# liuyuan-pal/Gen6D

Measured on AMD Instinct MI355X. Metric: query images/sec (detect+select+3x refine), 64 ref views, higher is better.
Workload: dtype f32

## Files before the change

### gen6d_amd/lib.py

```python
import ctypes as C
import os

_HERE = os.path.dirname(os.path.abspath(__file__))
LIB_PATH = os.path.join(_HERE, "libgen6d_hip.so")

G6D_ERRORS = {-1: "G6D_EINVAL", -2: "G6D_ENOSPC", -3: "G6D_ELAUNCH"}


class G6dWinoSeg(C.Structure):
    _fields_ = [("in_", C.c_void_p), ("out_full", C.c_void_p), ("out_pool", C.c_void_p),
                ("N", C.c_int32), ("H", C.c_int32), ("W", C.c_int32), ("ld_in", C.c_int32), ("ld_full", C.c_int32), ("ld_pool", C.c_int32)]


class G6dConv16Seg(C.Structure):
    _fields_ = [("in_", C.c_void_p), ("out_full", C.c_void_p), ("out_pool", C.c_void_p),
                ("N", C.c_int32), ("D", C.c_int32), ("H", C.c_int32), ("W", C.c_int32), ("ld_in", C.c_int32), ("ld_full", C.c_int32),
                ("ld_pool", C.c_int32)]


class G6dRange16(C.Structure):
    _fields_ = [("exps", C.c_void_p), ("rec", C.c_void_p), ("slot_in", C.c_int32), ("slot_out", C.c_int32)]


class G6dCorrSeg(C.Structure):
# ... 77 lines not shown
    "g6d_conv16_direct_plan": [_P, _I, _I, _P, _I, _I, _I, _I, _I, _I, _P, _I],
    "g6d_affine_split16_to": [_P, _I, _P, _P, _I, _I, _I, _I, _I, _I, _I, _P, _I, _I, _I, _I, _P, _P],
    "g6d_upsample_bilinear_split16": [_P, _I, _P, _P, _I, _I, _I, _I, _I, _I, _P, _I, _I, _I, _I, _P, _P],
    "g6d_l2norm_split16": [_P, _I, _I, _I, _P, _I, _P, _P],
    "g6d_vgg_conv1_pool_nhwc_norm": [_P, _I, _I, _I, _P, _P, _I, _I, _P, _P, _P, _P],
    "g6d_wino_conv3x3": [_P, _I, _I, _I, _I, _I, _P, _P, _I, _I, _P, _I, _P, _I, _P, C.c_size_t, _P],
    "g6d_wino_conv3x3_multi": [_P, _I, _I, _P, _P, _I, _I, _P, C.c_size_t, _P],
    "g6d_wino16_conv3x3_multi": [_P, _I, _I, _P, _P, _I, _I, _I, _P, C.c_size_t, _P],
    "g6d_wino43_conv3x3_multi": [_P, _I, _I, _P, _P, _I, _I, _P, C.c_size_t, _P],
    "g6d_corr2d_wino43_multi": [_P, _I, _I, _P, _I, _I, _P, C.c_size_t, _P],
    "g6d_l2norm_rows": [_P, _I, _I, _I, _P],
    "g6d_nchw_to_nhwc": [_P, _I, _I, _I, _I, _I, _P, _I, _P],
    "g6d_selector_ref_sums": [_P, _I, _I, _I, _P, _P, _P],
    "g6d_selector_prod_affine": [_P, _P, _P, _I, _I, _I, _D, _P, _P, _P],
    "g6d_selector_scan": [_P, _P, _I, _I, _I, _P, _P, _P],
    "g6d_selector_levels": [_I, _I, _P, _P, _P, _P, _P, _I, _I, _I, _D, _P, _P, _P, _P, _P],
    "g6d_refiner_volume": [_P, _P, _P, _P, _I, _I, _I, _I, _I, _I, _I, _P, _P, _P],
    "g6d_refiner_volume_kp": [_P, _P, _P, _P, _P, _P, _I, _I, _I, _I, _I, _I, _I, _P, _P, _I, _P],
    "g6d_refiner_volume_kp_pairs": [_P, _P, _P, _P, _P, _P, _I, _I, _I, _I, _I, _I, _I, _P, _P, _I, _P, _P, _P],
    "g6d_detector_assemble": [_P, _P, _P, _I, _I, _I, C.POINTER(C.c_float), _F, _I, _I, _I, _I, _P, _I, _P],
    "g6d_detector_score_mlp_max": [_P, _I, _I, _I, _P, _P, _P, _P, _P, _P],
    "g6d_detector_decode": [_P, _I, _P, _I, _P, _I, _I, _I, _I, _P, _I, _P],
    "g6d_resize_bilinear_pyramid": [_P, _I, _I, _I, _I, C.POINTER(C.c_int), C.POINTER(C.c_int), C.POINTER(C.c_void_p), _P],
    "g6d_zero_bytes": [_P, C.c_size_t, _P],
    "g6d_vps_norm": [_P, _I, _P, _I, _I, _I, _P],
    "g6d_max_an_add": [_P, _I, _I, _I, _I, _P, _P, _I, _I, _P],
    "g6d_attention": [_P, _P, _P, _I, _I, _I, _I, _P, _I, _I, _P],
    "g6d_layernorm": [_P, _I, _I, _I, _P, _P, _F, _P, _I, _P],
    "g6d_affine_act_add": [_P, _I, _P, _P, _I, _P, _I, _I, _I, _P, _I, _I, _P],
    "g6d_linear_gemv": [_P, _I, _I, _P, _P, _I, _I, _P, _P],
    "g6d_linear_gemv_batch": [_P, _I, _I, _P, _P, _I, _I, _P, _P, C.c_size_t, _P],
    "g6d_chain_crop_from_detection": [_P, _F, _P, _I, _P],
    "g6d_chain_pose_from_selection": [_P, _P, _P, _I, _P, _P, _P, _P, _P, _P, _I, _P],
    "g6d_chain_refine_prepare": [_P, _P, _P, _F, _F, _P, _P, _I, _I, _P, _P, _F, _P, _I, _P],
    "g6d_chain_refine_update": [_P, _P, _P, _P, _I, _P, _P, _I, _P],
    "g6d_warp_batch": [_P, _P, _P, _I, _I, _I, _I, _P, _P, _I, _I, _P],
    "g6d_warp_perspective": [_P, _I, _I, _I, C.POINTER(C.c_float), _P, _I, _I, _I, _F, _P],
    "g6d_track_gather": [_P, _P, _P, _P, _I, _P],
    "g6d_track_commit": [_P, _P, _P, _I, _P, _I, _F, _P, _P, _P, _P, _P, _I, _P],
    "g6d_track_gate": [_P, _P, _P, _P, _I, _P],
    "g6d_track_health": [_P, _P, _P, _P, _I, _I, _P, _I, _P, _D, _I, _D, _D, _D, _D, _D, _D, _P, _P, _P, _P, _I, _P],
    "g6d_track_verify": [_P, _P, _P, _P, _P, _D, _D, _D, _D, _I, _P, _P, _I, _P],
    "g6d_frame_ingest": [_P, _I, _P, _I, _I, _I, _P, _P],
    "g6d_sizeof_frame_desc": [],
    "g6d_frame_ingest_mesh": [_P, _P, _I, _P, _I, _I, _I, _P, _P],
    "g6d_sizeof_mesh_desc": [],
    "g6d_track_corners": [_P, _P, _P, _P, _P, _P, _I, _P],
    "g6d_frame_emit": [_P, _I, _P, _I, _I, _I, _P, _P, _P],
    "g6d_sizeof_sink_desc": [],
    "g6d_frame_emit_source": [_P, _I, _P, _I, _P, _P, _I, _I, _I, _I, _P],
    "g6d_frame_crop": [_P, _P, _P, _I, _I, _I, _P, _P, _I, _I, _P],
    "g6d_frame_ingest_area": [_P, _P, _I, _P, _I, _I, _I, _P, _P],
    "g6d_frame_crop_area": [_P, _P, _P, _I, _I, _I, _P, _P, _I, _I, _I, _P],
}

_lib = None


def load():
    global _lib
    if _lib is not None:
        return _lib
    if not os.path.exists(LIB_PATH):
        raise RuntimeError(f"{LIB_PATH} is missing: build it with `python __graft_entry__.py` "
                           "(make -C gen6d_amd/csrc). There is no fallback path.")
    import torch
    lib = C.CDLL(LIB_PATH)
    for name, args in SIGNATURES.items():
        fn = getattr(lib, name)
        fn.argtypes = args
        fn.restype = C.c_int
    lib.g6d_abi_version.restype = C.c_int
    lib.g6d_sizeof_conv_desc.restype = C.c_int
    if lib.g6d_sizeof_conv_desc() != C.sizeof(G6dConv):
        raise RuntimeError("libgen6d_hip.so: G6dConv layout differs from the ctypes binding (stale build?)")
    if lib.g6d_sizeof_frame_desc() != C.sizeof(G6dFrame):
        raise RuntimeError("libgen6d_hip.so: G6dFrame layout differs from the ctypes binding (stale build?)")
    if lib.g6d_sizeof_mesh_desc() != C.sizeof(G6dMesh):
        raise RuntimeError("libgen6d_hip.so: G6dMesh layout differs from the ctypes binding (stale build?)")
    if lib.g6d_sizeof_sink_desc() != C.sizeof(G6dSink):
        raise RuntimeError("libgen6d_hip.so: G6dSink layout differs from the ctypes binding (stale build?)")
    lib.g6d_last_error.restype = C.c_char_p
    lib.g6d_set_knob.argtypes, lib.g6d_set_knob.restype = [C.c_char_p, C.c_double], C.c_int
    lib.g6d_get_knob.argtypes, lib.g6d_get_knob.restype = [C.c_char_p], C.c_double
    lib.g6d_reset_knobs.argtypes, lib.g6d_reset_knobs.restype = [], None
    _lib = lib
    return lib


def set_knob(name, value):
    check(load().g6d_set_knob(name.encode(), float(value)), f"g6d_set_knob({name})")


def get_knob(name):
    return load().g6d_get_knob(name.encode())


def reset_knobs():
    load().g6d_reset_knobs()


def check(rc, what):
    if rc != 0:
        msg = load().g6d_last_error().decode()
        raise RuntimeError(f"{what} failed: {G6D_ERRORS.get(rc, rc)} ({msg})")
```

### gen6d_amd/network/detector.py

```python
import numpy as np
import torch
import torch.nn.functional as F

from .. import ops, parallel, specs
from .backbone import (is_16bit, pack_trunk, trunk_features, trunk_features_multi, trunk_route, winograd43_corr_filters,
                       winograd43_corr_filters_padded)
from .params import ParamBank, fold_vgg

_TAPS = ("c5", "c7_pre", "p7")
MAX_BATCH = 16


class Detector(ParamBank):
    default_cfg = {
        "vgg_score_stats": [[36.264317, 13.151907], [13910.291, 5345.965], [829.70807, 387.98788]],
        "vgg_score_max": 10,
        "detection_scales": [-1.0, -0.5, 0.0, 0.5],
        "train_feats": False,
    }

    def __init__(self, cfg):
        self.cfg = {**self.default_cfg, **cfg}
        super().__init__(specs.detector_rows())
        if len(self.cfg["detection_scales"]) != 4:
            raise NotImplementedError("score_conv expects 3 levels x 4 detection scales (12 channels)")
        self.pool_ratio = 8
        self.ref_center_feats = None
        self.ref_wino15_43 = None
        self.ref_wino7_43 = None
        self._corr16 = {}
        self.ref_shape = None
        self.rank, self.world, self.group = 0, 1, None
        self.sharded = False

    def set_shard(self, rank, world, group=None, force_collectives=False):
        self.rank, self.world, self.group = int(rank), int(world), group
        self.sharded = self.world > 1 or bool(force_collectives)

    def _pack(self):
        if self._packed is None:
            pk = {"vgg": pack_trunk(fold_vgg(self, "backbone.features"))}
            w0, b0 = self.conv_w("score_conv.0")
            w1, b1 = self.conv_w("score_conv.2")
            pk["mlp"] = (w0.reshape(64, 12).contiguous(), b0, w1.reshape(64, 64).contiguous(), b1)
            heads = ("score_predict", "scale_predict", "offset_predict")
            l0 = [self.conv_w(f"{h}.0") for h in heads]
            pk["h0"] = (torch.cat([w for w, _ in l0], 0).contiguous(), torch.cat([b for _, b in l0], 0).contiguous())
            pk["h1"] = [self.conv_w(f"{h}.2") for h in heads]
            l2 = [self.conv_w(f"{h}.4") for h in heads]
            w4 = torch.zeros((sum(w.shape[0] for w, _ in l2), 9, 192), dtype=torch.float32, device=l2[0][0].device)
            row = 0
            for i, (w, _) in enumerate(l2):
                w4[row:row + w.shape[0], :, 64 * i:64 * i + 64] = w
                row += w.shape[0]
            pk["h2"] = (w4.contiguous(), torch.cat([b for _, b in l2], 0).contiguous())
            self._packed = pk
        return self._packed

    def extract_feats(self, imgs):
        return trunk_features(self._pack()["vgg"], imgs, _TAPS, False)

    def load_impl(self, ref_imgs):
        b, e = parallel.shard_range(ref_imgs.shape[0], self.rank, self.world)
        if e == b:
            raise ValueError("more ranks than reference views")
        ref_imgs = F.interpolate(ref_imgs[b:e], size=(120, 120))
        feats = self.extract_feats(ref_imgs)
        self.ref_center_feats = [f.reshape(f.shape[0], f.shape[2] * f.shape[3], 512).contiguous() for f in feats]
        self.ref_ksize = [f.shape[2] for f in feats]
        self._corr16 = {}
        self.ref_shape = [120, 120]
        wino43 = self.ref_center_feats[0].shape[0] % 32 == 0
        self.ref_wino15_43 = winograd43_corr_filters(self.ref_center_feats[0], 15) if wino43 else None
        self.ref_wino7_43 = winograd43_corr_filters_padded(self.ref_center_feats[1], 7)[0] if wino43 else None

    def _corr16_filters(self, level, mode):
        if (level, mode) not in self._corr16:
            self._corr16[level, mode] = ops.corr16_pack(self.ref_center_feats[level], mode)
        return self._corr16[level, mode]

    def corr_routes(self, hq, wq):
        sizes = [self._scale_size(hq, wq, sc) for sc in self.cfg["detection_scales"]]
        trunk16 = trunk_route(self._pack()["vgg"], sizes, _TAPS, f43=True, pairs=self.pairs_on) == "direct"
        rfn = self.ref_center_feats[0].shape[0]
        routes = []
        for k in self.ref_ksize:
            if k in (15, 7) and trunk16 and rfn == 32:
                routes.append("corr16")
            elif k in (15, 7) and rfn % 32 == 0 and not ops.MATH_MODE:
                routes.append("wino43")
            else:
                routes.append("patch" if rfn <= 32 else "conv")
        return routes

    def _scores_one_scale(self, que_img, scale_idx, stacked, hs, ws):
        self._scores_from_feats(self.extract_feats(que_img), scale_idx, stacked, hs, ws)

    def _scores_from_pyramid(self, feats, routes, scale_ids, stacked, hs, ws):
        rfn = self.ref_center_feats[0].shape[0]
        dev = stacked.device
        qn = feats[0][0].shape[0]
        maps = [[None] * 3 for _ in feats]
        for l, (wref, k, route) in enumerate(zip(self.ref_center_feats, self.ref_ksize, routes)):
            xs = [f[l] for f in feats]
            assert is_16bit(xs[0]) == (route == "corr16"), "the trunk did not hand the level over in the format of its route"
            if route == "corr16":
                mode = 3 if len(xs[0].shape) == 5 else (1 if xs[0].dtype == torch.bfloat16 else 2)
                filt = self._corr16_filters(l, mode)
                outs = [torch.empty((qn, 1, x.shape[1], x.shape[2], rfn), dtype=torch.float32, device=dev) for x in xs]
                ops.corr16_multi(xs, filt, outs)
                for i, o in enumerate(outs):
                    maps[i][l] = o.reshape(qn * o.shape[2] * o.shape[3], rfn)
                continue
            lo = min(x.data_ptr() for x in xs)
            hi = max(x.data_ptr() + x.numel() * 4 for x in xs)
            if hi - lo >= (1 << 31) or not all(x.is_contiguous() for x in xs):
                seg = ops.alloc_like_segments([tuple(x.shape) for x in xs], dev)
                for d_, x in zip(seg, xs):
                    d_.copy_(x)
                xs = seg
            if route == "conv":
                outs = [torch.empty((qn, 1, x.shape[2], x.shape[3], rfn), dtype=torch.float32, device=dev) for x in xs]
                for x, o in zip(xs, outs):
                    ops.conv(x, wref, None, o, ksize=(1, k, k), pad=(0, k // 2, k // 2))
            else:
                outs = ops.alloc_like_segments([(qn, 1, x.shape[2], x.shape[3], rfn) for x in xs], dev)
                if route == "patch":
                    ops.corr2d_patch_multi(xs, wref, outs, k)
                elif k == 15:
                    ops.corr2d_wino43_multi([x.contiguous() for x in xs], self.ref_wino15_43, outs, 5)
                else:
                    ops.corr2d_wino43_multi([x.contiguous() for x in xs], self.ref_wino7_43, outs, 3, k_true=7)
            for i, o in enumerate(outs):
                maps[i][l] = o.reshape(qn * o.shape[2] * o.shape[3], rfn)
        for f, si, m in zip(feats, scale_ids, maps):
            hc, wc = (f[0].shape[1], f[0].shape[2]) if is_16bit(f[0]) else (f[0].shape[2], f[0].shape[3])
            ops.detector_assemble(m[0], m[1], m[2], hc, wc, self.cfg["vgg_score_stats"],
                                  float(self.cfg["vgg_score_max"]), hs, ws, si, stacked, batch=qn)

    def _scores_from_feats(self, feats, scale_idx, stacked, hs, ws):
        x0, x1, x2 = feats
        rfn = self.ref_center_feats[0].shape[0]
        qn = x0.shape[0]
        maps = []
        for x, wref, k in zip((x0, x1, x2), self.ref_center_feats, self.ref_ksize):
            _, _, h, w, _ = x.shape
            o = torch.empty((qn, 1, h, w, rfn), dtype=torch.float32, device=x.device)
            if k >= 7 and rfn <= 32 and qn == 1:
                ops.corr2d_patch(x, wref, o, k)
            else:
                ops.conv(x, wref, None, o, ksize=(1, k, k), pad=(0, k // 2, k // 2))
            maps.append(o.reshape(qn * h * w, rfn))
        hc, wc = x0.shape[2], x0.shape[3]
        ops.detector_assemble(maps[0], maps[1], maps[2], hc, wc, self.cfg["vgg_score_stats"],
                              float(self.cfg["vgg_score_max"]), hs, ws, scale_idx, stacked, batch=qn)

    @staticmethod
    def _scale_size(hq, wq, scale):
        ht, wt = int(np.round(hq * 2 ** scale)), int(np.round(wq * 2 ** scale))
        if ht % 32 != 0: ht = (ht // 32 + 1) * 32
        if wt % 32 != 0: wt = (wt // 32 + 1) * 32
        return ht, wt

    def _detect_batch(self, que_imgs, multi=True):
        pk = self._pack()
        qn, _, hq, wq = que_imgs.shape
        hs, ws = hq // 8, wq // 8
        dev = que_imgs.device
        rfn = self.ref_center_feats[0].shape[0]
        P = hs * ws
        stacked = torch.empty((qn * P, rfn, 12), dtype=torch.float32, device=dev)
        def resized(scale):
            return F.interpolate(que_imgs, size=self._scale_size(hq, wq, scale), mode="bilinear")

        order = sorted(enumerate(self.cfg["detection_scales"]), key=lambda t: -t[1])
        if multi:
            pyr = ops.resize_bilinear_pyramid(que_imgs, [self._scale_size(hq, wq, sc) for _, sc in order])
            routes = self.corr_routes(hq, wq)
            t16 = tuple(tap for tap, r in zip(_TAPS, routes) if r == "corr16")
            feats = trunk_features_multi(pk["vgg"], pyr, _TAPS, f43=True, taps16=t16, rng=self._pair_rng(), pairs=self.pairs_on)
            self._scores_from_pyramid(feats, routes, [si for si, _ in order], stacked, hs, ws)
        else:
            ops.fork_join([(lambda si=si, sc=sc: self._scores_one_scale(resized(sc), si, stacked, hs, ws)) for si, sc in order], dev)
        feats = ops.detector_score_mlp_max(stacked, *pk["mlp"])
        if self.sharded:
            parallel.all_reduce_(feats, "max", self.group)
        k3, p3 = (1, 3, 3), (0, 1, 1)
        a = torch.empty((qn, 1, hs, ws, 192), dtype=torch.float32, device=dev)
        ops.conv(feats.view(qn, 1, hs, ws, 64), pk["h0"][0], pk["h0"][1], a, ksize=k3, pad=p3, out_act=1)
        b = torch.empty_like(a)
        o4 = torch.empty((qn, 1, hs, ws, 4), dtype=torch.float32, device=dev)
        for i in range(3):
            w1, b1 = pk["h1"][i]
            ops.conv(a[..., 64 * i:64 * i + 64], w1, b1, b[..., 64 * i:64 * i + 64], ksize=k3, pad=p3, out_act=1)
        ops.conv(b, pk["h2"][0], pk["h2"][1], o4, ksize=k3, pad=p3)
        o4 = o4.view(qn * P, 4)
        res = ops.detector_decode(o4[:, 0:1], o4[:, 2:4], o4[:, 1:2], hs, ws, self.pool_ratio, batch=qn)
        return o4.view(qn, hs, ws, 4), res.view(qn, 5), (hs, ws)

    def detect_impl(self, *a, **k):
        with ops.math_mode(self.cfg.get("math_mode"), inherit_if_none=True):
            return self._detect_impl_fp(*a, **k)

    def _detect_impl_fp(self, que_imgs):
        outs, results = [], []
        _, _, hq, wq = que_imgs.shape
        per_query = sum(self._scale_size(hq, wq, sc)[0] * self._scale_size(hq, wq, sc)[1] for sc in self.cfg["detection_scales"]) // 4 * 64
        step = max(1, min(MAX_BATCH, ((1 << 29) - 1) // per_query))
        multi = per_query < (1 << 29)
        for q0 in range(0, que_imgs.shape[0], step):
            o4, res, _ = self._detect_batch(que_imgs[q0:q0 + step].contiguous(), multi)
            outs.append(o4.permute(0, 3, 1, 2))
            results.append(res)
        o = ops.cat1(outs, 0)
        r = ops.cat1(results, 0)
        return {"scores": o[:, 0:1], "select_pr_scale": o[:, 1:2], "select_pr_offset": o[:, 2:4],
                "que_select_id": r[:, 3:5].round().long(), "pool_ratio": self.pool_ratio,
                "positions": r[:, 0:2], "scales": r[:, 2]}

    def forward(self, data):
        self.load_impl(data["ref_imgs_info"]["imgs"])
        return self.detect_impl(data["que_imgs_info"]["imgs"])

    @staticmethod
    def parse_detection(scores, scales, offsets, pool_ratio):
        qn, _, hs, ws = scores.shape
        flat = torch.argmax(scores.flatten(1), 1)
        sy, sx = flat // ws, flat % ws
        ar = torch.arange(qn, device=scores.device)
        pos = (torch.stack([sx, sy], -1) + offsets[ar, :, sy, sx] + 0.5) * pool_ratio - 0.5
        return pos, 2 ** scales[ar, 0, sy, sx]
# ... 12 lines not shown
```

### gen6d_amd/ops.py

```python
import ctypes as C
import math

import numpy as np
import torch

from . import lib as _lib

_WS = {}
WORKSPACE_BYTES = 96 << 20
MATH_MODE = 0
_MATH_NAMES = {"fp32": 0, "f32": 0, "bf16": 1, "fp16": 2, "f16": 2, 0: 0, 1: 1, 2: 2, None: 0}


class math_mode:

    def __init__(self, mode, inherit_if_none=False):
        self.mode = None if (mode is None and inherit_if_none) else _MATH_NAMES[mode]

    def __enter__(self):
        global MATH_MODE
        self.prev = MATH_MODE
        if self.mode is not None:
            MATH_MODE = self.mode
        return self
# ... 907 lines not shown
    rc = _lib.load().g6d_conv16_direct_plan(seg, 1, Cin, C.c_void_p(any_), 2 if D else 1, Cout, 3 if D else 1, code, 0, int(mode),
                                            C.c_void_p(any_ if stats_rows else 0), int(stats_rows))
    return rc if rc >= 0 else None


def corr16_pack(w_taps, mode):
    co, taps, ci = w_taps.shape
    if co != 32 or ci % 32:
        raise ValueError("corr16_pack: 32 references and Cin % 32 == 0 expected")
    acc_scale = 1.0
    if mode == 3:
        hi, lo, acc_scale = _split_hi_lo(w_taps)
        x = torch.stack([hi, lo], 0).reshape(2, 32, taps, ci // 16, 2, 8)
        x = x.permute(3, 2, 0, 4, 1, 5).contiguous()
    else:
        x = w_taps.to(_T16[mode]).reshape(32, taps, ci // 32, 2, 2, 8)
        x = x.permute(2, 1, 3, 4, 0, 5).contiguous()
    k = int(round(taps ** 0.5))
    f = Conv16Filters(x.reshape(-1), 1, mode, acc_scale, co, taps, ci)
    f.k = k
    return f


def corr16_multi(xs, filt, outs):
    xs, table_in, slot_in = _pair_inputs(xs)
    if table_in is not None and filt.mode != 3:
        raise ValueError("corr16_multi: PairMaps need pair filters (mode 3)")
    ra = _range_arg(table_in, slot_in, None)
    _need_gpu(filt.data, *xs, *outs)
    mode, Cin = filt.mode, filt.Cin
    pair = mode == 3
    segs = (_lib.G6dConv16Seg * len(xs))()
    flops, sizes, nbytes = 0.0, [], 2.0 * filt.data.numel()
    for i, (x, o) in enumerate(zip(xs, outs)):
        if x.dtype != _T16[mode] or not x.is_contiguous() or x.dim() != (5 if pair else 4) or x.shape[-1] != Cin or not o.is_contiguous() \
                or o.dtype != torch.float32 or o.shape[-1] != 32:
            raise ValueError("corr16_multi: dense 16-bit channels-last inputs and dense fp32 outputs with 32 channels expected")
        N, H, W = x.shape[0], x.shape[1], x.shape[2]
        if o.numel() != N * H * W * 32:
            raise ValueError("corr16_multi: output shape mismatch")
        segs[i] = _lib.G6dConv16Seg(in_=x.data_ptr(), out_full=o.data_ptr(), out_pool=None, N=N, D=1, H=H, W=W, ld_in=(2 if pair else 1) * Cin,
                                    ld_full=32, ld_pool=0)
        flops += 2.0 * N * H * W * 32 * filt.taps * Cin
        nbytes += x.numel() * 2.0 + o.numel() * 4.0
        sizes.append(f"{N}x{H}x{W}")
    _timed(PROFILE is not None,
           lambda: _lib.check(_lib.load().g6d_corr16_multi_ex(segs, len(xs), Cin, _ptr(filt.data), float(filt.acc_scale), 32, int(filt.k), int(mode), ra,
                                                             _stream()), "g6d_corr16_multi"),
           lambda e0, e1: PROFILE.append((flops, e0, e1, f"{'conv16x3' if pair else 'conv16'} corr in={'+'.join(sizes)}x{Cin} out=32 k={filt.k}x{filt.k}",
                                          nbytes, flops)))
    return outs


def l2norm_rows(x):
    _need_gpu(x)
    Cc = x.shape[-1]
    if x.dtype == torch.float32 and x.dim() == 2 and x.stride(1) == 1 and not x.is_contiguous():
        _lib.check(_lib.load().g6d_l2norm_rows(_ptr(x), x.shape[0], Cc, x.stride(0), _stream()), "g6d_l2norm_rows")
        return x
    if x.dtype != torch.float32 or not x.is_contiguous():
        raise ValueError("l2norm_rows: contiguous float32 expected")
    _lib.check(_lib.load().g6d_l2norm_rows(_ptr(x), x.numel() // Cc, Cc, Cc, _stream()), "g6d_l2norm_rows")
    return x


def nchw_to_nhwc(x, out, l2norm):
    _need_gpu(x, out)
    if not x.is_contiguous() or x.dtype != torch.float32:
        raise ValueError("nchw_to_nhwc: x must be contiguous float32 NCHW")
    N, Cc, H, W = x.shape
    _, _, Ho, Wo, Co, ld_out = _cl5(out, "nchw_to_nhwc.out")
    if (Ho, Wo, Co) != (H, W, Cc):
        raise ValueError("nchw_to_nhwc: shape mismatch")
    _lib.check(_lib.load().g6d_nchw_to_nhwc(_ptr(x), N, Cc, H, W, int(l2norm), _ptr(out), ld_out, _stream()), "g6d_nchw_to_nhwc")
    return out


def selector_ref_sums(refs):
    _need_gpu(refs)
    D, HW, Cc = refs.shape
    r1 = torch.empty((HW, Cc), dtype=torch.float64, device=refs.device)
    r2 = torch.empty_like(r1)
    _lib.check(_lib.load().g6d_selector_ref_sums(_ptr(refs.contiguous()), D, HW, Cc, _ptr(r1), _ptr(r2), _stream()),
               "g6d_selector_ref_sums")
    return r1, r2


def selector_prod_affine(que, r1, r2, D, eps=1e-5):
    _need_gpu(que, r1, r2)
    HW, Cc = que.shape
    scale = torch.empty((1, Cc), dtype=torch.float32, device=que.device)
    shift = torch.empty_like(scale)
    _lib.check(_lib.load().g6d_selector_prod_affine(_ptr(que), _ptr(r1), _ptr(r2), D, HW, Cc, float(eps), _ptr(scale),
                                                   _ptr(shift), _stream()), "g6d_selector_prod_affine")
    return scale, shift


def selector_scan(que, refs):
    _need_gpu(que, refs)
    D, HW, Cc = refs.shape
    if not (que.is_contiguous() and refs.is_contiguous()):
        raise ValueError("selector_scan: operands must be contiguous")
    smap = torch.empty((D, HW), dtype=torch.float32, device=que.device)
    vps = torch.empty((D,), dtype=torch.float32, device=que.device)
    _timed_hbm("selector_scan", 4.0 * (D * HW * Cc + HW * Cc + 2 * D * HW + D),
               lambda: _lib.check(_lib.load().g6d_selector_scan(_ptr(que), _ptr(refs), D, HW, Cc, _ptr(smap), _ptr(vps),
# ... 570 lines not shown
```

### include/gen6d_hip.h

```cpp
#ifndef GEN6D_HIP_H
#define GEN6D_HIP_H

#include <stddef.h>
#include <stdint.h>

#ifdef __cplusplus
extern "C" {
#endif

typedef void* g6d_stream_t;

enum {
  G6D_OK = 0,
  G6D_EINVAL = -1,
  G6D_ENOSPC = -2,
  G6D_ELAUNCH = -3
};

int g6d_abi_version(void);
const char* g6d_last_error(void);

int g6d_set_knob(const char* name, double value);
double g6d_get_knob(const char* name);
void g6d_reset_knobs(void);
// ... 248 lines not shown
  int32_t pitch0, pitch1;
  int32_t width, height;
  int32_t format;
  int32_t rotate;
  int32_t matrix;
  int32_t slot;
  int32_t out_w, out_h;
  float   K[9];
} G6dFrame;
int g6d_frame_ingest(const G6dFrame* frames, int n, uint8_t* out, int B, int H, int W, float* K_out, g6d_stream_t stream);
int g6d_sizeof_frame_desc(void);

typedef struct G6dMesh {
  const int32_t* nodes;
  int32_t nx, ny;
  int32_t step_log2;
  int32_t reserved;
} G6dMesh;
int g6d_frame_ingest_mesh(const G6dFrame* frames, const G6dMesh* meshes, int n, uint8_t* out, int B, int H, int W, float* K_out,
                          g6d_stream_t stream);
int g6d_sizeof_mesh_desc(void);

int g6d_frame_ingest_area(const G6dFrame* frames, const G6dMesh* meshes , int n, uint8_t* out, int B, int H, int W,
                          float* K_out, g6d_stream_t stream);

int g6d_track_corners(const float* table, const float* K, const int* slot_stream, const float* box, int32_t* pts, int32_t* valid,
                      int batch, g6d_stream_t stream);
typedef struct G6dSink {
  void* plane0;
  void* plane1;
  int32_t pitch0, pitch1;
  int32_t width, height;
  int32_t format;
  int32_t matrix;
  int32_t slot;
  int32_t pic_w, pic_h;
  int32_t thickness, dot_radius;
  int32_t line_rgb, dot_rgb;
  int32_t box;
} G6dSink;
int g6d_frame_emit(const G6dSink* sinks, int n, const uint8_t* imgs, int B, int H, int W, const int32_t* pts, const int32_t* valid,
                   g6d_stream_t stream);
int g6d_sizeof_sink_desc(void);

int g6d_frame_emit_source(const G6dSink* sinks, int n, const G6dFrame* frames, int nf, const int32_t* pts, const int32_t* valid, int sets,
                          int B, int max_w, int max_h, g6d_stream_t stream);

int g6d_frame_crop(const G6dFrame* frames, const int32_t* rec, const uint8_t* imgs, int B, int H, int W, const float* hinv, float* dst,
                   int dh, int dw, g6d_stream_t stream);

int g6d_frame_crop_area(const G6dFrame* frames, const int32_t* rec, const uint8_t* imgs, int B, int H, int W, const float* hinv, float* dst,
                        int dh, int dw, int max_n, g6d_stream_t stream);

#ifdef __cplusplus
}
#endif
#endif
```

Measured before the change: 366.2.

## Add FFT-based correlation route for 15x15 detector level

Adds an FFT correlation path for the k=15 reference correlation. Query maps are cut into overlapping 32x32 tiles and transformed with a register radix-2 FFT. They are multiplied against precomputed reference spectra using an fp32 MFMA per-bin GEMM, then inverse-transformed. It is meant to replace direct or Winograd spatial correlation, whose cost grows with the 225 taps, when there are enough queries (threshold 4). The trade is large spectrum and product buffers in memory traffic and possible fp32 rounding differences.

```diff
diff --git a/gen6d_amd/csrc/corr_fft.hip b/gen6d_amd/csrc/corr_fft.hip
--- /dev/null
+++ b/gen6d_amd/csrc/corr_fft.hip
@@ -0,0 +1,293 @@
+#include "g6d_common.h"
+#include "corr_fft_plan.h"
+
+namespace {
+
+constexpr int T = 32, HB = T / 2 + 1;
+constexpr int CG = 32;
+constexpr int RS = HB * 2 * CG;
+constexpr int FWD_LDS = T * RS * 4;
+constexpr int NT = 512;
+
+struct CfftSeg { const float* in; float* out; int ld_in, ld_out; };
+struct CfftParams {
+  cfft::Plan plan;
+  CfftSeg seg[cfft::MAX_SEG];
+  int Cin;
+  float* X;
+  const float* Y;
+};
+
+__host__ __device__ constexpr double tw_c8(int k) {
+  constexpr double c[9] = {1.0, 0.98078528040323043, 0.92387953251128674, 0.83146961230254524, 0.70710678118654752,
+                           0.55557023301960218, 0.38268343236508977, 0.19509032201612825, 0.0};
+  return c[k];
+}
+__host__ __device__ constexpr double tw_cos(int k) { return k <= 8 ? tw_c8(k) : -tw_c8(16 - k); }
+__host__ __device__ constexpr double tw_sin(int k) { return k <= 8 ? tw_c8(8 - k) : tw_c8(k - 8); }
+__host__ __device__ constexpr int br5(int k) { return ((k & 1) << 4) | ((k & 2) << 2) | (k & 4) | ((k & 8) >> 2) | ((k & 16) >> 4); }
+
+__device__ __forceinline__ void fft32(float (&re)[T], float (&im)[T]) {
+#pragma unroll
+  for (int h = 16; h >= 1; h >>= 1) {
+#pragma unroll
+    for (int b = 0; b < T; b += 2 * h) {
+#pragma unroll
+      for (int j = 0; j < h; ++j) {
+        const int k = j * (16 / h);
+        const float c = (float)tw_cos(k), s = (float)tw_sin(k);
+        const float ur = re[b + j], ui = im[b + j], vr = re[b + j + h], vi = im[b + j + h];
+        re[b + j] = ur + vr; im[b + j] = ui + vi;
+        const float dr = ur - vr, di = ui - vi;
+        if (k == 0) { re[b + j + h] = dr; im[b + j + h] = di; }
+        else if (k == 8) { re[b + j + h] = di; im[b + j + h] = -dr; }
+        else { re[b + j + h] = dr * c + di * s; im[b + j + h] = di * c - dr * s; }
+      }
+    }
+  }
+}
+
+__global__ __launch_bounds__(NT) void corrfft_fwd_kernel(const CfftParams p) {
+  extern __shared__ __attribute__((aligned(16))) float L[];
+  const int tid = threadIdx.x, c = tid & (CG - 1), g = tid >> 5;
+  const int tile = blockIdx.x, c0 = blockIdx.y * CG;
+  const cfft::Tile t = cfft::tile_of(p.plan, tile);
+  const cfft::SegPlan& sp = p.plan.seg[t.seg];
+  const CfftSeg& sg = p.seg[t.seg];
+  const int H = sp.H, W = sp.W, wy = cfft::window_y(p.plan, t), wx = cfft::window_x(p.plan, t);
+  float re[T], im[T];
+  {
+    const int ya = wy + 2 * g, yb = ya + 1;
+    const bool oka = ya >= 0 && ya < H, okb = yb >= 0 && yb < H;
+    const float* img = sg.in + (size_t)t.n * H * W * sg.ld_in + c0 + c;
+#pragma unroll
+    for (int x = 0; x < T; ++x) {
+      const int xx = wx + x;
+      const bool okx = xx >= 0 && xx < W;
+      re[x] = oka && okx ? img[((size_t)ya * W + xx) * sg.ld_in] : 0.f;
+      im[x] = okb && okx ? img[((size_t)yb * W + xx) * sg.ld_in] : 0.f;
+    }
+  }
+  fft32(re, im);
+  {
+    float* ra = L + (2 * g) * RS + c;
+    float* rb = ra + RS;
+#pragma unroll
+    for (int k = 0; k < HB; ++k) {
+      const int a = br5(k), b = br5((T - k) & (T - 1));
+      ra[k * 64] = 0.5f * (re[a] + re[b]); ra[k * 64 + 32] = 0.5f * (im[a] - im[b]);
+      rb[k * 64] = 0.5f * (im[a] + im[b]); rb[k * 64 + 32] = 0.5f * (re[b] - re[a]);
+    }
+  }
+  __syncthreads();
+  if (g == 0) {
+#pragma unroll
+    for (int y = 0; y < T; ++y) { re[y] = L[y * RS + c]; im[y] = L[y * RS + 16 * 64 + c]; }
+  } else {
+#pragma unroll
+    for (int y = 0; y < T; ++y) { re[y] = L[y * RS + g * 64 + c]; im[y] = L[y * RS + g * 64 + 32 + c]; }
+  }
+  fft32(re, im);
+  if (g == 0) {
+#pragma unroll
+    for (int k = 0; k < T; ++k) {
+      const int a = br5(k), b = br5((T - k) & (T - 1));
+      L[k * RS + c] = 0.5f * (re[a] + re[b]); L[k * RS + 32 + c] = 0.5f * (im[a] - im[b]);
+      L[k * RS + 16 * 64 + c] = 0.5f * (im[a] + im[b]); L[k * RS + 16 * 64 + 32 + c] = 0.5f * (re[b] - re[a]);
+    }
+  } else {
+#pragma unroll
+    for (int k = 0; k < T; ++k) { L[k * RS + g * 64 + c] = re[br5(k)]; L[k * RS + g * 64 + 32 + c] = im[br5(k)]; }
+  }
+  __syncthreads();
+  const size_t tiles = (size_t)p.plan.tiles;
+#pragma unroll 1
+  for (int i = tid; i < T * HB * 16; i += NT) {
+    const int q = i & 7, pl = (i >> 3) & 1, bin = i >> 4, ky = bin / HB, kx = bin - ky * HB;
+    const f32x4 v = *reinterpret_cast<const f32x4*>(L + ky * RS + kx * 64 + pl * 32 + 4 * q);
+    *reinterpret_cast<f32x4*>(p.X + (((size_t)bin * tiles + tile) * 2 + pl) * p.Cin + c0 + 4 * q) = v;
+  }
+}
+
+constexpr int GEMM_NT = 128, GEMM_BM = 128;
+struct CfftGemm { const float* X; const float* B; float* Y; int M, bins, K2, mblocks; };
+
+__global__ __launch_bounds__(GEMM_NT) void corrfft_gemm_kernel(const CfftGemm p) {
+  const int b = blockIdx.x, xcd = b & 7, s = b >> 3;
+  const int bin = xcd + 8 * (s / p.mblocks), mb = s % p.mblocks;
+  if (bin >= p.bins) return;
+  const int lane = threadIdx.x & 63, wv = threadIdx.x >> 6, r = lane & 31, h = lane >> 5;
+  const int m0 = mb * GEMM_BM + wv * 64;
+  if (m0 >= p.M) return;
+  const int K2 = p.K2;
+  const float* A0 = p.X + ((size_t)bin * p.M + min(m0 + r, p.M - 1)) * K2 + 16 * h;
+  const float* A1 = p.X + ((size_t)bin * p.M + min(m0 + 32 + r, p.M - 1)) * K2 + 16 * h;
+  const float* Bp = p.B + ((size_t)bin * K2 + 16 * h) * 64 + r;
+  f32x16 acc[2][2];
+#pragma unroll
+  for (int i = 0; i < 2; ++i)
+#pragma unroll
+    for (int n = 0; n < 2; ++n)
+#pragma unroll
+      for (int q = 0; q < 16; ++q) acc[i][n][q] = 0.f;
+  f32x4 a0[2][4], a1[2][4];
+  float b0[2][16], b1[2][16];
+  auto load = [&](int k0, f32x4 (&x0)[4], f32x4 (&x1)[4], float (&y0)[16], float (&y1)[16]) {
+#pragma unroll
+    for (int j = 0; j < 4; ++j) {
+      x0[j] = *reinterpret_cast<const f32x4*>(A0 + k0 + 4 * j);
+      x1[j] = *reinterpret_cast<const f32x4*>(A1 + k0 + 4 * j);
+    }
+#pragma unroll
+    for (int e = 0; e < 16; ++e) { y0[e] = Bp[(size_t)(k0 + e) * 64]; y1[e] = Bp[(size_t)(k0 + e) * 64 + 32]; }
+  };
+  auto mac = [&](const f32x4 (&x0)[4], const f32x4 (&x1)[4], const float (&y0)[16], const float (&y1)[16]) {
+#pragma unroll
+    for (int e = 0; e < 16; ++e) {
+      const float u0 = x0[e >> 2][e & 3], u1 = x1[e >> 2][e & 3];
+      acc[0][0] = __builtin_amdgcn_mfma_f32_32x32x2f32(u0, y0[e], acc[0][0], 0, 0, 0);
+      acc[0][1] = __builtin_amdgcn_mfma_f32_32x32x2f32(u0, y1[e], acc[0][1], 0, 0, 0);
+      acc[1][0] = __builtin_amdgcn_mfma_f32_32x32x2f32(u1, y0[e], acc[1][0], 0, 0, 0);
+      acc[1][1] = __builtin_amdgcn_mfma_f32_32x32x2f32(u1, y1[e], acc[1][1], 0, 0, 0);
+    }
+  };
+  load(0, a0[0], a1[0], b0[0], b1[0]);
+#pragma unroll 1
+  for (int k0 = 0; k0 < K2; k0 += 64) {
+    load(k0 + 32, a0[1], a1[1], b0[1], b1[1]);
+    mac(a0[0], a1[0], b0[0], b1[0]);
+    if (k0 + 64 < K2) load(k0 + 64, a0[0], a1[0], b0[0], b1[0]);
+    mac(a0[1], a1[1], b0[1], b1[1]);
+  }
+  float* Yb = p.Y + (size_t)bin * p.M * 64 + r;
+#pragma unroll
+  for (int i = 0; i < 2; ++i)
+#pragma unroll
+    for (int q = 0; q < 16; ++q) {
+      const int row = m0 + 32 * i + (q & 3) + 8 * (q >> 2) + 4 * h;
+      if (row < p.M) { Yb[(size_t)row * 64] = acc[i][0][q]; Yb[(size_t)row * 64 + 32] = acc[i][1][q]; }
+    }
+}
+
+constexpr int INV_ROWS = 18;
+constexpr int INV_LDS = INV_ROWS * RS * 4;
+
+__global__ __launch_bounds__(NT) void corrfft_inv_kernel(const CfftParams p) {
+  extern __shared__ __attribute__((aligned(16))) float L[];
+  const int tid = threadIdx.x, r = tid & (CG - 1), g = tid >> 5;
+  const int tile = blockIdx.x, V = p.plan.V;
+  const cfft::Tile t = cfft::tile_of(p.plan, tile);
+  const cfft::SegPlan& sp = p.plan.seg[t.seg];
+  const CfftSeg& sg = p.seg[t.seg];
+  const size_t bs = (size_t)p.plan.tiles * 64;
+  const float* Y = p.Y + (size_t)tile * 64 + r;
+  float re[T], im[T];
+  if (g == 0) {
+#pragma unroll
+    for (int k = 0; k < T; ++k) {
+      const float* y0 = Y + (size_t)(k * HB) * bs;
+      const float* y16 = Y + (size_t)(k * HB + 16) * bs;
+      re[k] = y0[0] - y16[32]; im[k] = y0[32] + y16[0];
+    }
+  } else {
+#pragma unroll
+    for (int k = 0; k < T; ++k) {
+      const float* y = Y + (size_t)(k * HB + g) * bs;
+      re[k] = y[0]; im[k] = y[32];
+    }
+  }
+  fft32(im, re);
+  if (g == 0) {
+#pragma unroll
+    for (int y = 0; y < INV_ROWS; ++y) {
+      L[y * RS + r] = re[br5(y)]; L[y * RS + 32 + r] = 0.f;
+      L[y * RS + 16 * 64 + r] = im[br5(y)]; L[y * RS + 16 * 64 + 32 + r] = 0.f;
+    }
+  } else {
+#pragma unroll
+    for (int y = 0; y < INV_ROWS; ++y) { L[y * RS + g * 64 + r] = re[br5(y)]; L[y * RS + g * 64 + 32 + r] = im[br5(y)]; }
+  }
+  __syncthreads();
+  if (2 * g >= V) return;
+  const float* ga = L + (2 * g) * RS + r;
+  const float* gb = ga + RS;
+#pragma unroll
+  for (int k = 0; k < HB; ++k) {
+    const float ar = ga[k * 64], ai = ga[k * 64 + 32], br = gb[k * 64], bi = gb[k * 64 + 32];
+    re[k] = ar - bi; im[k] = ai + br;
+    if (k > 0 && k < T / 2) { re[T - k] = ar + bi; im[T - k] = br - ai; }
+  }
+  fft32(im, re);
+  const int H = sp.H, W = sp.W, ya = t.y0 + 2 * g;
+  const float sc = 1.f / (T * T);
+  float* o = sg.out + (size_t)t.n * H * W * sg.ld_out + r;
+#pragma unroll
+  for (int x = 0; x < INV_ROWS; ++x) {
+    const int xx = t.x0 + x;
+    if (x < V && xx < W) {
+      if (ya < H) o[((size_t)ya * W + xx) * sg.ld_out] = re[br5(x)] * sc;
+      if (ya + 1 < H) o[((size_t)(ya + 1) * W + xx) * sg.ld_out] = im[br5(x)] * sc;
+    }
+  }
+}
+
+int cfft_params(CfftParams& p, const char* what, const G6dCorrSeg* segs, int nseg, int C, int k, int Tw, bool fwd) {
+  if (!segs || nseg < 1 || nseg > cfft::MAX_SEG) { g6d_set_error("corr_fft: 1..4 segments expected"); return G6D_EINVAL; }
+  if (Tw != T || k != 15) { g6d_set_error("corr_fft: the kernels are built for T = 32, k = 15"); return G6D_EINVAL; }
+  int N[cfft::MAX_SEG], H[cfft::MAX_SEG], W[cfft::MAX_SEG];
+  for (int i = 0; i < nseg; ++i) { N[i] = segs[i].N; H[i] = segs[i].H; W[i] = segs[i].W; }
+  if (!cfft::make_plan(p.plan, Tw, k, nseg, N, H, W) || p.plan.V > INV_ROWS || (p.plan.V & 1)) { g6d_set_error("corr_fft: bad map sizes"); return G6D_EINVAL; }
+  for (int i = 0; i < nseg; ++i) {
+    const G6dCorrSeg& s = segs[i];
+    const bool ok = fwd ? (s.in && s.ld_in >= C && !(s.ld_in & 3) && g6d_aligned16(s.in)) : (s.out && s.ld_out >= C);
+    if (!ok) { g6d_set_error(what); return G6D_EINVAL; }
+    p.seg[i] = CfftSeg{s.in, s.out, s.ld_in, s.ld_out};
+  }
+  return G6D_OK;
+}
+}
+
+extern "C" int g6d_corr_fft_plan(const G6dCorrSeg* segs, int nseg, int Cin, int Cout, int k, int Tw, int64_t* out) {
+  if (!segs || !out || nseg < 1 || nseg > cfft::MAX_SEG || Cin < 1 || Cout < 1) { g6d_set_error("corr_fft_plan: bad arguments"); return G6D_EINVAL; }
+  int N[cfft::MAX_SEG], H[cfft::MAX_SEG], W[cfft::MAX_SEG], one[cfft::MAX_SEG];
+  for (int i = 0; i < nseg; ++i) { N[i] = segs[i].N; H[i] = segs[i].H; W[i] = segs[i].W; one[i] = 1; }
+  cfft::Plan p, q;
+  if (!cfft::make_plan(p, Tw, k, nseg, N, H, W) || !cfft::make_plan(q, Tw, k, nseg, one, H, W)) { g6d_set_error("corr_fft_plan: bad sizes"); return G6D_EINVAL; }
+  out[0] = p.tiles; out[1] = p.bins; out[2] = p.V;
+  out[3] = cfft::spectrum_bytes(Tw, p.tiles, Cin); out[4] = cfft::product_bytes(Tw, p.tiles, Cout); out[5] = cfft::filter_bytes(Tw, Cin, Cout);
+  out[6] = q.tiles;
+  out[7] = cfft::chunk_queries(Tw, q.tiles, Cin, 1 << 16);
+  return G6D_OK;
+}
+
+extern "C" int g6d_corr_fft_fwd(const G6dCorrSeg* segs, int nseg, int Cin, int k, int Tw, float* X, g6d_stream_t stream) {
+  CfftParams p = {};
+  if (int rc = cfft_params(p, "corr_fft_fwd: bad segment (fp32 channels-last maps, 16-byte aligned, ld_in % 4 == 0)", segs, nseg, Cin, k, Tw, true)) return rc;
+  if (!X || !g6d_aligned16(X) || Cin % CG) { g6d_set_error("corr_fft_fwd: Cin % 32 == 0 and an aligned spectrum expected"); return G6D_EINVAL; }
+  if (cfft::spectrum_bytes(Tw, p.plan.tiles, Cin) >= (1ll << 31)) { g6d_set_error("corr_fft_fwd: spectrum beyond 2 GB, launch fewer queries"); return G6D_ENOSPC; }
+  p.Cin = Cin; p.X = X;
+  g6d_allow_lds(reinterpret_cast<const void*>(&corrfft_fwd_kernel), FWD_LDS);
+  hipLaunchKernelGGL(corrfft_fwd_kernel, dim3(p.plan.tiles, Cin / CG), dim3(NT), FWD_LDS, static_cast<hipStream_t>(stream), p);
+  return g6d_check_launch("corr_fft_fwd");
+}
+
+extern "C" int g6d_corr_fft_gemm(const float* X, const float* B, float* Y, int tiles, int Cin, int Cout, int Tw, g6d_stream_t stream) {
+  if (!X || !B || !Y || tiles < 1 || Tw != T || Cout != 32 || Cin < 32 || Cin % 32 || !g6d_aligned16(X)) {
+    g6d_set_error("corr_fft_gemm: T = 32, 32 references, Cin % 32 == 0 expected"); return G6D_EINVAL;
+  }
+  if (cfft::spectrum_bytes(Tw, tiles, Cin) >= (1ll << 31)) { g6d_set_error("corr_fft_gemm: spectrum beyond 2 GB"); return G6D_ENOSPC; }
+  CfftGemm p = {X, B, Y, tiles, cfft::bins(Tw), 2 * Cin, (tiles + GEMM_BM - 1) / GEMM_BM};
+  static_assert(cfft::bins(T) % 8 == 0, "blocks of a bin stay on one XCD");
+  hipLaunchKernelGGL(corrfft_gemm_kernel, dim3(p.bins * p.mblocks), dim3(GEMM_NT), 0, static_cast<hipStream_t>(stream), p);
+  return g6d_check_launch("corr_fft_gemm");
+}
+
+extern "C" int g6d_corr_fft_inv(const G6dCorrSeg* segs, int nseg, int Cout, int k, int Tw, const float* Y, g6d_stream_t stream) {
+  CfftParams p = {};
+  if (int rc = cfft_params(p, "corr_fft_inv: bad segment (ld_out >= 32)", segs, nseg, Cout, k, Tw, false)) return rc;
+  if (!Y || Cout != CG) { g6d_set_error("corr_fft_inv: 32 references expected"); return G6D_EINVAL; }
+  p.Y = Y;
+  g6d_allow_lds(reinterpret_cast<const void*>(&corrfft_inv_kernel), INV_LDS);
+  hipLaunchKernelGGL(corrfft_inv_kernel, dim3(p.plan.tiles), dim3(NT), INV_LDS, static_cast<hipStream_t>(stream), p);
+  return g6d_check_launch("corr_fft_inv");
+}
diff --git a/gen6d_amd/csrc/corr_fft_plan.h b/gen6d_amd/csrc/corr_fft_plan.h
--- /dev/null
+++ b/gen6d_amd/csrc/corr_fft_plan.h
@@ -0,0 +1,64 @@
+#pragma once
+#include <stdint.h>
+
+#if defined(__HIPCC__) || defined(__CUDACC__)
+#define CFFT_HD __host__ __device__ inline
+#else
+#define CFFT_HD inline
+#endif
+
+namespace cfft {
+
+constexpr int MAX_SEG = 4;
+
+CFFT_HD constexpr bool valid_tk(int T, int K) { return (T == 32 || T == 64) && K >= 1 && (K & 1) && K < T; }
+CFFT_HD constexpr int valid_side(int T, int K) { return T - K + 1; }
+CFFT_HD constexpr int bins(int T) { return T * (T / 2 + 1); }
+
+struct SegPlan { int H, W, N, tiles_x, tiles_y, tpi, tile0; };
+struct Plan {
+  int T, K, V, bins, nseg, tiles;
+  SegPlan seg[MAX_SEG];
+};
+struct Tile { int seg, n, y0, x0; };
+
+CFFT_HD int ceil_div(int a, int b) { return (a + b - 1) / b; }
+
+CFFT_HD bool make_plan(Plan& p, int T, int K, int nseg, const int* N, const int* H, const int* W) {
+  if (!valid_tk(T, K) || nseg < 1 || nseg > MAX_SEG) return false;
+  p.T = T; p.K = K; p.V = valid_side(T, K); p.bins = bins(T); p.nseg = nseg;
+  int64_t tiles = 0;
+  for (int i = 0; i < nseg; ++i) {
+    if (N[i] < 1 || H[i] < 1 || W[i] < 1) return false;
+    SegPlan& s = p.seg[i];
+    s.H = H[i]; s.W = W[i]; s.N = N[i];
+    s.tiles_x = ceil_div(W[i], p.V); s.tiles_y = ceil_div(H[i], p.V);
+    s.tpi = s.tiles_x * s.tiles_y; s.tile0 = (int)tiles;
+    tiles += (int64_t)s.tpi * N[i];
+    if (tiles >= (1ll << 24)) return false;
+  }
+  p.tiles = (int)tiles;
+  return true;
+}
+
+CFFT_HD Tile tile_of(const Plan& p, int t) {
+  int si = 0;
+  for (int i = 1; i < p.nseg; ++i) if (t >= p.seg[i].tile0) si = i;
+  const SegPlan& s = p.seg[si];
+  const int l = t - s.tile0, n = l / s.tpi, r = l - n * s.tpi, ty = r / s.tiles_x, tx = r - ty * s.tiles_x;
+  return {si, n, ty * p.V, tx * p.V};
+}
+CFFT_HD int window_y(const Plan& p, const Tile& t) { return t.y0 - p.K / 2; }
+CFFT_HD int window_x(const Plan& p, const Tile& t) { return t.x0 - p.K / 2; }
+
+CFFT_HD int64_t spectrum_bytes(int T, int64_t tiles, int Cin) { return (int64_t)bins(T) * tiles * 2 * Cin * 4; }
+CFFT_HD int64_t product_bytes(int T, int64_t tiles, int R) { return (int64_t)bins(T) * tiles * 2 * R * 4; }
+CFFT_HD int64_t filter_bytes(int T, int Cin, int R) { return (int64_t)bins(T) * 2 * Cin * 2 * R * 4; }
+
+CFFT_HD int chunk_queries(int T, int tiles_per_query, int Cin, int want) {
+  int q = want;
+  while (q > 0 && spectrum_bytes(T, (int64_t)q * tiles_per_query, Cin) >= (1ll << 31)) --q;
+  return q;
+}
+
+}
diff --git a/gen6d_amd/lib.py b/gen6d_amd/lib.py
--- a/gen6d_amd/lib.py
+++ b/gen6d_amd/lib.py
@@ -153,6 +153,10 @@
     "g6d_frame_crop": [_P, _P, _P, _I, _I, _I, _P, _P, _I, _I, _P],
     "g6d_frame_ingest_area": [_P, _P, _I, _P, _I, _I, _I, _P, _P],
     "g6d_frame_crop_area": [_P, _P, _P, _I, _I, _I, _P, _P, _I, _I, _I, _P],
+    "g6d_corr_fft_plan": [_P, _I, _I, _I, _I, _I, _P],
+    "g6d_corr_fft_fwd": [_P, _I, _I, _I, _I, _P, _P],
+    "g6d_corr_fft_gemm": [_P, _P, _P, _I, _I, _I, _I, _P],
+    "g6d_corr_fft_inv": [_P, _I, _I, _I, _I, _P, _P],
 }
 
 _lib = None
diff --git a/gen6d_amd/network/detector.py b/gen6d_amd/network/detector.py
--- a/gen6d_amd/network/detector.py
+++ b/gen6d_amd/network/detector.py
@@ -9,6 +9,7 @@
 
 _TAPS = ("c5", "c7_pre", "p7")
 MAX_BATCH = 16
+CORR_FFT_MIN_QUERIES = 4
 
 
 class Detector(ParamBank):
@@ -29,6 +30,7 @@
         self.ref_wino15_43 = None
         self.ref_wino7_43 = None
         self._corr16 = {}
+        self._corr_fft = None
         self.ref_shape = None
         self.rank, self.world, self.group = 0, 1, None
         self.sharded = False
@@ -69,6 +71,7 @@
         self.ref_center_feats = [f.reshape(f.shape[0], f.shape[2] * f.shape[3], 512).contiguous() for f in feats]
         self.ref_ksize = [f.shape[2] for f in feats]
         self._corr16 = {}
+        self._corr_fft = None
         self.ref_shape = [120, 120]
         wino43 = self.ref_center_feats[0].shape[0] % 32 == 0
         self.ref_wino15_43 = winograd43_corr_filters(self.ref_center_feats[0], 15) if wino43 else None
@@ -79,14 +82,21 @@
             self._corr16[level, mode] = ops.corr16_pack(self.ref_center_feats[level], mode)
         return self._corr16[level, mode]
 
-    def corr_routes(self, hq, wq):
+    def _corr_fft_filters(self):
+        if self._corr_fft is None:
+            self._corr_fft = ops.corr_fft_spectra(self.ref_center_feats[0])
+        return self._corr_fft
+
+    def corr_routes(self, hq, wq, qn=1):
         sizes = [self._scale_size(hq, wq, sc) for sc in self.cfg["detection_scales"]]
         trunk16 = trunk_route(self._pack()["vgg"], sizes, _TAPS, f43=True, pairs=self.pairs_on) == "direct"
         rfn = self.ref_center_feats[0].shape[0]
         routes = []
         for k in self.ref_ksize:
             if k in (15, 7) and trunk16 and rfn == 32:
-                routes.append("corr16")
+                want = self.cfg.get("corr_fft")
+                fft = k == 15 and not ops.MATH_MODE and not self.sharded and want is not False and (want or qn >= CORR_FFT_MIN_QUERIES)
+                routes.append("fft" if fft else "corr16")
             elif k in (15, 7) and rfn % 32 == 0 and not ops.MATH_MODE:
                 routes.append("wino43")
             else:
@@ -109,6 +119,12 @@
                 filt = self._corr16_filters(l, mode)
                 outs = [torch.empty((qn, 1, x.shape[1], x.shape[2], rfn), dtype=torch.float32, device=dev) for x in xs]
                 ops.corr16_multi(xs, filt, outs)
+                for i, o in enumerate(outs):
+                    maps[i][l] = o.reshape(qn * o.shape[2] * o.shape[3], rfn)
+                continue
+            if route == "fft":
+                outs = [torch.empty((qn, 1, x.shape[2], x.shape[3], rfn), dtype=torch.float32, device=dev) for x in xs]
+                ops.corr_fft_multi([x.contiguous() for x in xs], self._corr_fft_filters(), outs)
                 for i, o in enumerate(outs):
                     maps[i][l] = o.reshape(qn * o.shape[2] * o.shape[3], rfn)
                 continue
@@ -176,7 +192,7 @@
         order = sorted(enumerate(self.cfg["detection_scales"]), key=lambda t: -t[1])
         if multi:
             pyr = ops.resize_bilinear_pyramid(que_imgs, [self._scale_size(hq, wq, sc) for _, sc in order])
-            routes = self.corr_routes(hq, wq)
+            routes = self.corr_routes(hq, wq, qn)
             t16 = tuple(tap for tap, r in zip(_TAPS, routes) if r == "corr16")
             feats = trunk_features_multi(pk["vgg"], pyr, _TAPS, f43=True, taps16=t16, rng=self._pair_rng(), pairs=self.pairs_on)
             self._scores_from_pyramid(feats, routes, [si for si, _ in order], stacked, hs, ws)
diff --git a/gen6d_amd/ops.py b/gen6d_amd/ops.py
--- a/gen6d_amd/ops.py
+++ b/gen6d_amd/ops.py
@@ -983,6 +983,130 @@
     return outs
 
 
+CORR_FFT_T = 32
+CORR_FFT_CHUNK = 4
+
+
+def _corr_fft_segs(xs, outs, Cin, what):
+    n = len(xs if xs is not None else outs)
+    if not 1 <= n <= 4:
+        raise ValueError(f"{what}: 1..4 segments expected")
+    segs = (_lib.G6dCorrSeg * n)()
+    for i in range(n):
+        x = xs[i] if xs is not None else None
+        o = outs[i] if outs is not None else None
+        for t, ch in ((x, Cin), (o, 32)):
+            if t is not None and (t.dtype != torch.float32 or not t.is_contiguous() or t.dim() not in (4, 5) or t.shape[-1] != ch
+                                  or (t.dim() == 5 and t.shape[1] != 1)):
+                raise ValueError(f"{what}: dense fp32 channels-last maps [N,(1,)H,W,{ch}] expected")
+        ref = x if x is not None else o
+        N, H, W = ref.shape[0], ref.shape[-3], ref.shape[-2]
+        if x is not None and o is not None and (o.shape[0], o.shape[-3], o.shape[-2]) != (N, H, W):
+            raise ValueError(f"{what}: output shape mismatch")
+        segs[i] = _lib.G6dCorrSeg(in_=x.data_ptr() if x is not None else None, out=o.data_ptr() if o is not None else None, H=H, W=W,
+                                  ld_in=Cin, ld_out=32, N=N, reserved_=0)
+    return segs
+
+
+def corr_fft_plan(sizes, Cin, Cout=32, k=15, T=CORR_FFT_T):
+    segs = (_lib.G6dCorrSeg * len(sizes))()
+    for i, (N, H, W) in enumerate(sizes):
+        segs[i] = _lib.G6dCorrSeg(in_=None, out=None, H=H, W=W, ld_in=Cin, ld_out=Cout, N=N, reserved_=0)
+    out = (C.c_int64 * 8)()
+    _lib.check(_lib.load().g6d_corr_fft_plan(segs, len(sizes), Cin, Cout, k, T, out), "g6d_corr_fft_plan")
+    keys = ("tiles", "bins", "V", "spectrum_bytes", "product_bytes", "filter_bytes", "tiles_per_query", "max_queries")
+    return dict(zip(keys, (int(v) for v in out)))
+
+
+class CorrFftSpectra:
+
+    def __init__(self, data, Cin, k, T):
+        self.data, self.Cin, self.k, self.T = data, Cin, k, T
+
+
+def corr_fft_spectra(w_taps, T=CORR_FFT_T):
+    R, taps, Cin = w_taps.shape
+    k = int(round(taps ** 0.5))
+    if R != 32 or k * k != taps or k >= T:
+        raise ValueError("corr_fft_spectra: [32, k*k, Cin] filters with k < T expected")
+    w = w_taps.detach().to("cpu", torch.float64).reshape(R, k, k, Cin).permute(0, 3, 1, 2)
+    Wf = torch.fft.rfft2(torch.nn.functional.pad(w, (0, T - k, 0, T - k)))
+    Wr = Wf.real.permute(2, 3, 1, 0).reshape(-1, Cin, R)
+    Wi = Wf.imag.permute(2, 3, 1, 0).reshape(-1, Cin, R)
+    B = torch.cat([torch.cat([Wr, -Wi], 2), torch.cat([Wi, Wr], 2)], 1).to(torch.float32).contiguous()
+    return CorrFftSpectra(B.to(w_taps.device), Cin, k, T)
+
+
+def corr_fft_fwd(xs, X, k=15, T=CORR_FFT_T):
+    Cin = xs[0].shape[-1]
+    _need_gpu(X, *xs)
+    segs = _corr_fft_segs(xs, None, Cin, "corr_fft_fwd")
+    plan = corr_fft_plan([(s.N, s.H, s.W) for s in segs], Cin, 32, k, T)
+    if X.dtype != torch.float32 or not X.is_contiguous() or X.numel() * 4 < plan["spectrum_bytes"]:
+        raise ValueError("corr_fft_fwd: the spectrum buffer is smaller than [bins][tiles][2][Cin] fp32")
+    _lib.check(_lib.load().g6d_corr_fft_fwd(segs, len(xs), Cin, k, T, _ptr(X), _stream()), "g6d_corr_fft_fwd")
+    return X
+
+
+def corr_fft_gemm(X, B, Y, tiles, Cin, T=CORR_FFT_T):
+    _need_gpu(X, B, Y)
+    bins = T * (T // 2 + 1)
+    if X.numel() < bins * tiles * 2 * Cin or B.numel() != bins * 2 * Cin * 64 or Y.numel() < bins * tiles * 64 \
+            or any(t.dtype != torch.float32 or not t.is_contiguous() for t in (X, B, Y)):
+        raise ValueError("corr_fft_gemm: fp32 X [bins][tiles][2 Cin], B' [bins][2 Cin][64], Y [bins][tiles][64] expected")
+    _lib.check(_lib.load().g6d_corr_fft_gemm(_ptr(X), _ptr(B), _ptr(Y), int(tiles), int(Cin), 32, T, _stream()), "g6d_corr_fft_gemm")
+    return Y
+
+
+def corr_fft_inv(Y, outs, k=15, T=CORR_FFT_T):
+    _need_gpu(Y, *outs)
+    segs = _corr_fft_segs(None, outs, 32, "corr_fft_inv")
+    plan = corr_fft_plan([(s.N, s.H, s.W) for s in segs], 32, 32, k, T)
+    if Y.dtype != torch.float32 or not Y.is_contiguous() or Y.numel() * 4 < plan["product_bytes"]:
+        raise ValueError("corr_fft_inv: the product buffer is smaller than [bins][tiles][2][32] fp32")
+    _lib.check(_lib.load().g6d_corr_fft_inv(segs, len(outs), 32, k, T, _ptr(Y), _stream()), "g6d_corr_fft_inv")
+    return outs
+
+
+def corr_fft_multi(xs, spectra, outs, chunk=None):
+    Cin, k, T = spectra.Cin, spectra.k, spectra.T
+    N = xs[0].shape[0]
+    if any(x.shape[0] != N or x.shape[-1] != Cin for x in xs) or len(xs) != len(outs):
+        raise ValueError("corr_fft_multi: every segment holds the same queries and Cin channels")
+    _need_gpu(spectra.data, *xs, *outs)
+    _corr_fft_segs(xs, outs, Cin, "corr_fft_multi")
+    one = corr_fft_plan([(1, x.shape[-3], x.shape[-2]) for x in xs], Cin, 32, k, T)
+    qc = min(N, one["max_queries"], int(chunk or CORR_FFT_CHUNK))
+    if qc < 1:
+        raise ValueError("corr_fft_multi: one query's spectrum passes 2^31 bytes")
+    dev = xs[0].device
+    tiles_max = one["tiles_per_query"] * qc
+    bins = one["bins"]
+    X = torch.empty(bins * tiles_max * 2 * Cin, dtype=torch.float32, device=dev)
+    Y = torch.empty(bins * tiles_max * 64, dtype=torch.float32, device=dev)
+    on = PROFILE is not None
+    log2t = math.log2(T)
+    for q0 in range(0, N, qc):
+        q1 = min(N, q0 + qc)
+        tiles = one["tiles_per_query"] * (q1 - q0)
+        xc, oc = [x[q0:q1] for x in xs], [o[q0:q1] for o in outs]
+        sizes = "+".join(f"{q1 - q0}x{x.shape[-3]}x{x.shape[-2]}" for x in xs)
+        f_fft = 5.0 * T * log2t
+        fl_fwd = tiles * Cin * (T / 2 + T / 2) * f_fft
+        fl_gemm = 2.0 * bins * tiles * (2 * Cin) * 64
+        fl_inv = tiles * 32 * (T / 2 + (T - k + 1) / 2) * f_fft
+        act = sum(x.numel() for x in xc) * 4.0
+        _timed(on, lambda: corr_fft_fwd(xc, X, k, T),
+               lambda e0, e1: PROFILE.append((fl_fwd, e0, e1, f"corr_fft fwd in={sizes}x{Cin} T={T}", act + 4.0 * bins * tiles * 2 * Cin, fl_fwd)))
+        _timed(on, lambda: corr_fft_gemm(X, spectra.data, Y, tiles, Cin, T),
+               lambda e0, e1: PROFILE.append((fl_gemm, e0, e1, f"corr_fft gemm bins={bins} M={tiles} K={2 * Cin} N=64",
+                                              4.0 * (bins * tiles * (2 * Cin + 64) + spectra.data.numel()), fl_gemm)))
+        _timed(on, lambda: corr_fft_inv(Y, oc, k, T),
+               lambda e0, e1: PROFILE.append((fl_inv, e0, e1, f"corr_fft inv out={sizes}x32 T={T}",
+                                              4.0 * bins * tiles * 64 + sum(o.numel() for o in oc) * 4.0, fl_inv)))
+    return outs
+
+
 def l2norm_rows(x):
     _need_gpu(x)
     Cc = x.shape[-1]
diff --git a/include/gen6d_hip.h b/include/gen6d_hip.h
--- a/include/gen6d_hip.h
+++ b/include/gen6d_hip.h
@@ -324,6 +324,11 @@
 int g6d_frame_crop_area(const G6dFrame* frames, const int32_t* rec, const uint8_t* imgs, int B, int H, int W, const float* hinv, float* dst,
                         int dh, int dw, int max_n, g6d_stream_t stream);
 
+int g6d_corr_fft_plan(const G6dCorrSeg* segs, int nseg, int Cin, int Cout, int k, int T, int64_t* out);
+int g6d_corr_fft_fwd(const G6dCorrSeg* segs, int nseg, int Cin, int k, int T, float* X, g6d_stream_t stream);
+int g6d_corr_fft_gemm(const float* X, const float* B, float* Y, int tiles, int Cin, int Cout, int T, g6d_stream_t stream);
+int g6d_corr_fft_inv(const G6dCorrSeg* segs, int nseg, int Cout, int k, int T, const float* Y, g6d_stream_t stream);
+
 #ifdef __cplusplus
 }
 #endif
```

Result: faster. 394.4, median of 6 (+7.7%).
